# SheffieldML/GPy

Hardware: AMD Instinct MI355X
Metric: exact-GP log_lik+grad iters/sec (higher is better)
Workload: dtype f64; 1 GPU; BASELINE configs[2]: matern52 ARD exact GP, one GPRegression.parameters_changed, N=16384 D=32 Dy=1 per GPU; N=16384, D=32, kernel=matern52, ARD=True, parallelism=replicas x1

## Files before the change

### gpy_amd/_lib.py

```python
import ctypes
import os
import subprocess

import numpy as np
from numpy.ctypeslib import ndpointer

_HERE = os.path.dirname(os.path.abspath(__file__))
LIB_PATH = os.environ.get("MI355GP_LIB") or os.path.join(_HERE, "libmi355gp.so")
CSRC = os.path.join(_HERE, "csrc")

KIND_IDS = {"rbf": 0, "matern52": 1, "matern32": 2, "exponential": 3, "white": 4, "bias": 5, "ratquad": 6, "stdperiodic": 7,
            "coregionalize": 8, "linear": 9, "mlp": 10, "poly": 11, "cosine": 12, "sinc": 13, "expquadcosine": 14}


def ard_id(kind, ARD):
    if kind == "coregionalize":
        return int(ARD)
    return int(ARD) & 3 if kind == "stdperiodic" else int(bool(ARD))


class Part(ctypes.Structure):
    _fields_ = [("kind", ctypes.c_int), ("ard", ctypes.c_int), ("n_active", ctypes.c_int),
                ("active_dims", ctypes.POINTER(ctypes.c_int)), ("theta", ctypes.POINTER(ctypes.c_double)),
                ("term", ctypes.c_int)]
# ... 118 lines not shown
    "mi355gp_sparse_get_predict_ms": [_vp, _c_dp],
    "mi355gp_sparse_fetch_dLdKnm": [_vp, _i64, _i64, _dp],
    "mi355gp_sparse_attach_comm": [_vp, _ci, _ci, _str],
    "mi355gp_sparse_attach_loopback": [_vp, _ci, _ci, _ci],
    "mi355gp_sparse_fetch": [_vp, _ci, _dp],
    "mi355gp_sparse_get_profile": [_vp, _dp],
    "mi355gp_svgp_forward": [_vp, _ci, _parts, _dp, _i64, _dp, _dp, _ci, _cd, _dp, _dp, _dp, _c_dp],
    "mi355gp_svgp_backward": [_vp, _dp, _dp] + [_c_dp] * 5,
    "mi355gp_svgp_predict": [_vp, _ci, _parts, _c_dp, _i64, _ci] + [_c_dp] * 4,
    "mi355gp_pep_inference": [_vp, _ci, _parts, _dp, _i64, _cd, _cd, _cd, _dp] + [_c_dp] * 5,
    "mi355gp_pep_check_sigma": [_dp, _i64, _i64, _cd, _cd],
    "mi355gp_rbf_psi": [_ci, _cd, _dp, _ci, _dp, _i64, _dp, _dp, _i64, _ci] + [_c_dp] * 3,
    "mi355gp_rbf_psi_grad": [_ci, _cd, _dp, _ci, _dp, _i64, _dp, _dp, _i64, _ci] + [_c_dp] * 4 + [_dp] * 5,
    "mi355gp_bench_factor": [_ci, _i64, _ci, _c_dp, _c_dp, _c_dp],
    "mi355gp_dbg_ipc_selftest": [_str, _ci, _ci, _ci, _ci, _i64, _dp],
    "mi355gp_dbg_comm_selftest": [_ci, _str, _ci, _ci, _ci, _ci, _i64, _ci, _dp],
    "mi355gp_dbg_grid_multi": [_ci, _ci, _ci, _ci, _dp],
    "mi355gp_dbg_update_nt": [_ci, _ci, _ip, _ci, _ci, _dp],
    "mi355gp_dbg_update_rect": [_ci, _ci, _ci, _ip, _ci, _ci, _dp],
    "mi355gp_dbg_mfma": [_ci, _dp, _dp, _dp],
    "mi355gp_dbg_gemm": [_ci, _ci, _ci, _i64, _i64, _i64, _dp, _dp, _dp, _cd, _cd, _ci, _c_dp],
    "mi355gp_dbg_peaks": [_ci, _dp],
    "mi355gp_dbg_gemm_clock": [_c_dp, _c_dp],
    "mi355gp_dbg_cu_map": [_ci, _ci, _ci, ctypes.POINTER(ctypes.c_uint)],
    "mi355gp_dbg_pipe_share": [_ci, _dp],
    "mi355gp_dbg_graph_factor": [_ci, _i64, _ci, _dp],
    "mi355gp_dbg_persist": [_ci, _i64, _ci, _ci, _dp],
    "mi355gp_dbg_lauum_plan": [_ci, _ip, _ci, _ip],
    "mi355gp_dbg_persist_owners": [_ci, _ci, _ci, _ip, _ip],
    "mi355gp_dbg_mask_probe": [_ci, _ci, _ci, _dp],
}
EXPORTED = tuple(ABI)


def _opt(a):
    return None if a is None else a.ctypes.data_as(_c_dp)


def lib():
    global _lib
    if _lib is None:
        if not os.path.exists(LIB_PATH):
            build()
        L = ctypes.CDLL(LIB_PATH)
        for name, argtypes in ABI.items():
            getattr(L, name).argtypes = argtypes
        L.mi355gp_last_error.restype = L.mi355gp_version.restype = _str
        _lib = L
    return _lib


OPTIONS = {"profile": 0, "lookahead": 1, "tri_overlap": 2, "tri_min_nt": 3, "tri_h": 4, "tri_wgs": 5, "tri_half": 6,
           "part1_on_panel": 7, "nbo": 8, "solve_overlap": 9, "diag_excl_first": 10, "graph": 11, "persist": 12, "agg2": 13,
           "persist_test": 14, "persist_aborts": 15, "persist_skip": 16, "persist_sched": 17}


def last_error():
    return lib().mi355gp_last_error().decode()


def check(rc, what):
    if rc < 0:
        raise MI355GPError("%s failed (rc=%d): %s" % (what, rc, last_error()))
    return rc


def device_count():
    n = ctypes.c_int(0)
    lib().mi355gp_device_count(ctypes.byref(n))
    return n.value


def device_synchronize(device=0):
    require_device(device)
    check(lib().mi355gp_device_synchronize(int(device)), "mi355gp_device_synchronize")


def require_device(device=0):
    n = device_count()
    if device >= n:
        raise MI355GPError("no MI355X visible to HIP (device %d requested, %d present): the gpy_amd backend has "
                           "no CPU fallback" % (device, n))


def f64(a):
    return np.ascontiguousarray(a, dtype=np.float64)


def theta_vec(variance, lengthscale, ARD, D):
    ls = np.atleast_1d(np.asarray(lengthscale, dtype=np.float64)).ravel()
    if ARD:
        if ls.size == 1:
            ls = np.full(D, ls[0])
        assert ls.size == D, "ARD kernel needs one lengthscale per input dimension"
    else:
        assert ls.size == 1, "isotropic kernel has a single lengthscale"
    return np.concatenate([[float(np.asarray(variance).ravel()[0])], ls])


def _exact_result(out, ms, **arrays):
    res = dict(lml=out[OUT_LML], logdet=out[OUT_LOGDET], datafit=out[OUT_DATAFIT], dnoise=out[OUT_DNOISE],
               trKinv=out[OUT_TRKINV], **arrays)
    if ms is not None:
        res["stage_ms"] = dict(zip(STAGE_NAMES, ms[:len(STAGE_NAMES)]))
    return res


# ... 604 lines not shown
```

### gpy_amd/csrc/api.hip

```cpp
#include <cstdarg>
#include <cstdio>
#include <climits>
#include <string>
#include <vector>

#include "ctx.h"

static thread_local std::string g_err;

void mi355gp_set_error(const char* fmt, ...) {
    char buf[1024];
    va_list ap;
    va_start(ap, fmt);
    vsnprintf(buf, sizeof(buf), fmt, ap);
    va_end(ap);
    g_err = buf;
}

void apply_options(mi355gp_ctx* c) {
    FactorWs& w = c->ws;
    auto set = [&](int o, int* field) { if (c->opt[o] != INT_MIN) *field = c->opt[o]; };
    set(MI355GP_OPT_LOOKAHEAD, &w.lookahead);
    set(MI355GP_OPT_TRI_OVERLAP, &w.tri_overlap);
    set(MI355GP_OPT_TRI_MIN_NT, &w.tri_min_nt);
    set(MI355GP_OPT_TRI_H, &w.tri_h_override);
    set(MI355GP_OPT_TRI_WGS, &w.tri_wgs);
    set(MI355GP_OPT_TRI_HALF, &w.tri_half_ok);
    set(MI355GP_OPT_PART1_ON_PANEL, &w.part1_on_panel);
    set(MI355GP_OPT_NBO, &w.nbo_override);
    set(MI355GP_OPT_SOLVE_OVERLAP, &w.solve_overlap);
    set(MI355GP_OPT_DIAG_EXCL_FIRST, &w.diag_excl_first);
    set(MI355GP_OPT_PERSIST, &w.persist);
    set(MI355GP_OPT_AGG2, &w.agg2);
    if (c->opt[MI355GP_OPT_GRAPH] != INT_MIN) c->graph_enabled = c->opt[MI355GP_OPT_GRAPH] ? 1 : 0;
}

void drop_graph(mi355gp_ctx* c) {
    if (c->fgraph) (void)hipGraphExecDestroy(c->fgraph);
    c->fgraph = nullptr;
    c->fgraph_calls = 0;
}

void free_data(mi355gp_ctx* c) {
    drop_graph(c);
    c->parts.clear();
    double** ptrs[] = {&c->dX, &c->dR, &c->dNoise, &c->A, &c->B, &c->C, &c->Mbuf,
                       &c->dTmp, &c->dTrmvPart, &c->dGradPart, &c->dGradOut, &c->dPack, &c->dCoregPart};
    for (auto p : ptrs) {
        if (*p) (void)hipFree(*p);
        *p = nullptr;
    }
    if (c->hPack) (void)hipHostFree(c->hPack);
    c->hPack = nullptr;
    c->dAlpha = c->dScal = c->dDiag = c->dGradOutAll = nullptr;
    c->hIdx.clear();
    c->hIdxCol = -1;
    laplace_session_free(c->lap);
    c->lap = nullptr;
    c->lap_stage = 0;
    factor_ws_free(&c->ws);
    c->have_factor = c->have_kernel = false;
}

int ctx_prepare_parts(mi355gp_ctx* c, int nparts, const mi355gp_part* parts) {
    ARG_CHECK(nparts >= 1 && nparts <= 16 && parts, "between 1 and 16 kernel parts");
    if ((int)c->parts.size() != nparts) {
        c->parts.clear();
        c->parts.resize((size_t)nparts);
        for (auto& p : c->parts) HIP_CHECK(p.dXt.alloc((size_t)c->D * c->npad));
    }
    for (int i = 0; i < nparts; ++i) {
        mi355gp_ctx::Part& p = c->parts[(size_t)i];
        if (int rc = parse_part(parts[i], c->D, KS_STATIONARY | KS_STATIC | KS_EXT | KS_COREG | KS_LINEAR | KS_DOT | KS_OSC, "exact-GP path", &p)) return rc;
        if (p.coreg()) {
            const int col = p.kp.col;
            if (c->hIdxCol != col) {
                c->hIdx.resize((size_t)c->n);
                HIP_CHECK(hipMemcpy2D(c->hIdx.data(), sizeof(double), c->dX + col, sizeof(double) * c->D, sizeof(double), c->n,
                                      hipMemcpyDeviceToHost));
                c->hIdxCol = col;
            }
            if (int rc = coreg_check_index(c->hIdx.data(), c->n, 1, p.kp.ard, "training")) return rc;
            if (!c->dCoregPart) HIP_CHECK(hipMalloc(&c->dCoregPart, sizeof(double) * grad_num_blocks(c->n) * COREG_REC));
        }
        if (int rc = p.upload(c->st)) return rc;
    }
// ... 200 lines not shown
    }
    HIP_CHECK(hipMemcpyAsync(out, tmp, sizeof(double) * n * n, hipMemcpyDeviceToHost, st));
    HIP_CHECK(hipStreamSynchronize(st));
    return 0;
}

int mi355gp_set_option(mi355gp_ctx* c, int option, int value) {
    ARG_CHECK(c != nullptr, "mi355gp_set_option: NULL context");
    if (option == MI355GP_OPT_PROFILE) {
        c->ws.prof.on = (value != 0);
        c->ws.prof.mask = (value == 1) ? 0xffu : (unsigned)value >> 1;
        return 0;
    }
    if (option == MI355GP_OPT_PERSIST_TEST) {
#ifndef MI355GP_DIAG
        if (value != 0) {
            mi355gp_set_error("mi355gp_set_option: MI355GP_OPT_PERSIST_TEST is a test hook of the diagnostics build (libmi355gp_diag.so)");
            return -1;
        }
#endif
        c->ws.persist_test = value;
        if (value) c->ws.persist_skip = 0;
        drop_graph(c);
        return 0;
    }
    if (option < 0 || option >= MI355GP_OPT_NUM || option == MI355GP_OPT_PERSIST_ABORTS || option == MI355GP_OPT_PERSIST_SKIP ||
        option == MI355GP_OPT_PERSIST_SCHED) {
        mi355gp_set_error("mi355gp_set_option: unknown or read-only option %d", option);
        return -1;
    }
    if (option == MI355GP_OPT_LOOKAHEAD) value = (value == 0) ? 0 : 1;
    if (option == MI355GP_OPT_NBO && value > 0 && value % NB != 0) {
        mi355gp_set_error("mi355gp_set_option: NBO must be a multiple of %d", NB);
        return -1;
    }
    c->opt[option] = (value < 0) ? INT_MIN : value;
    if (value < 0) {
        FactorWs d;
#define env(name, dflt) diag_env_int(DIAG_ENV(name), dflt)
#define penv(name, dflt) diag_env_int(PRODUCT_ENV(name), dflt)
        switch (option) {
            case MI355GP_OPT_LOOKAHEAD: c->ws.lookahead = d.lookahead; break;
            case MI355GP_OPT_TRI_OVERLAP: c->ws.tri_overlap = penv("TRI_OVERLAP", d.tri_overlap) ? 1 : 0; break;
            case MI355GP_OPT_TRI_MIN_NT: c->ws.tri_min_nt = env("TRI_MIN_NT", d.tri_min_nt); break;
            case MI355GP_OPT_TRI_H: c->ws.tri_h_override = env("TRI_H", d.tri_h_override); break;
            case MI355GP_OPT_TRI_WGS: c->ws.tri_wgs = env("TRI_WGS", d.tri_wgs); break;
            case MI355GP_OPT_TRI_HALF: c->ws.tri_half_ok = env("TRI_HALF", d.tri_half_ok) ? 1 : 0; break;
            case MI355GP_OPT_PART1_ON_PANEL: c->ws.part1_on_panel = env("PART1_ON_PANEL", d.part1_on_panel) ? 1 : 0; break;
            case MI355GP_OPT_NBO: c->ws.nbo_override = env("NBO", d.nbo_override); break;
            case MI355GP_OPT_SOLVE_OVERLAP: c->ws.solve_overlap = env("SOLVE_OVERLAP", d.solve_overlap) ? 1 : 0; break;
            case MI355GP_OPT_DIAG_EXCL_FIRST: c->ws.diag_excl_first = env("DIAG_EXCL_FIRST", d.diag_excl_first) ? 1 : 0; break;
            case MI355GP_OPT_PERSIST: c->ws.persist = penv("PERSIST", d.persist); break;
            case MI355GP_OPT_AGG2: c->ws.agg2 = env("AGG2", d.agg2) ? 1 : 0; break;
            case MI355GP_OPT_GRAPH: c->graph_enabled = penv("GRAPH", 1) ? 1 : 0; break;
            default: break;
        }
#undef env
#undef penv
    }
    if (option == MI355GP_OPT_PERSIST) {
        c->ws.persist_auto_off = 0;
        c->ws.sched_force_steps = 0;
        c->ws.sched_np = c->ws.sched_ns = 0;
        c->ws.sched_state = (value < 0) ? 0 : 2;
    }
    apply_options(c);
    drop_graph(c);
    return 0;
}

int mi355gp_get_option(mi355gp_ctx* c, int option, int* value) {
    ARG_CHECK(c && value && option > MI355GP_OPT_PROFILE && option < MI355GP_OPT_NUM, "mi355gp_get_option: bad arguments");
    const FactorWs& w = c->ws;
    const int v[MI355GP_OPT_NUM] = {0, w.lookahead, w.tri_overlap, w.tri_min_nt, w.tri_h_override, w.tri_wgs, w.tri_half_ok,
                                    w.part1_on_panel, w.nbo_override, w.solve_overlap, w.diag_excl_first, c->graph_enabled,
                                    w.persist, w.agg2, w.persist_test, w.persist_aborts, w.persist_skip,
                                    w.sched_state == 2 ? ((w.persist_auto_off || !w.persist) ? 2 : 1) : 0};
    *value = v[option];
    return 0;
}

int mi355gp_get_profile(mi355gp_ctx* c, double* ms, double* flops, int* launches) {
    ARG_CHECK(c && ms && flops && launches, "mi355gp_get_profile: NULL argument");
    HIP_CHECK(hipSetDevice(c->device));
    HIP_CHECK(hipStreamSynchronize(c->st));
    if (c->ws.st_panel) HIP_CHECK(hipStreamSynchronize(c->ws.st_panel));
    if (c->ws.prof.collect(ms, flops, launches) != 0) {
        mi355gp_set_error("mi355gp_get_profile: event timing failed");
        return -5;
    }
    return 0;
}

}
```

### gpy_amd/csrc/factor.hip

```cpp
#include <cstdlib>
#include <mutex>
#include <vector>

#include "internal.h"

void KernelProf::begin(hipStream_t st, int fam, double flops) {
    open = on && ((mask >> fam) & 1u);
    if (!open) return;
    const size_t e0 = 2 * recs.size();
    while (pool.size() < e0 + 2) {
        hipEvent_t e;
        (void)hipEventCreate(&e);
        pool.push_back(e);
    }
    recs.push_back(Rec{fam, flops, e0});
    (void)hipEventRecord(pool[e0], st);
}

void KernelProf::end(hipStream_t st) {
    if (!open) return;
    open = false;
    (void)hipEventRecord(pool[recs.back().e0 + 1], st);
}

// ... 71 lines not shown
            void* touch = nullptr;
            if (hipMalloc(&touch, 256) == hipSuccess) {
                hipStream_t order[4] = {e.main, e.panel, e.tri, e.tri_half};
                for (hipStream_t s : order)
                    if (s) {
                        (void)hipMemsetAsync(touch, 0, 256, s);
                        (void)hipStreamSynchronize(s);
                    }
                (void)hipFree(touch);
            }
        }
        e.ready = true;
    }
    if (main) *main = e.main;
    if (panel) *panel = e.panel;
    if (tri) *tri = e.tri;
    if (tri_half) *tri_half = e.tri_half;
    return 0;
}

static bool lauum_plan_wanted(const FactorWs* ws, int nt);
static bool lauum_plan_build(FactorWs* ws, int nt);
int factor_ws_alloc(FactorWs* ws, long npad) {
    ws->nblk = npad / NB;
    HIP_CHECK(hipMalloc(&ws->dinv, sizeof(double) * ws->nblk * 8 * 256));
    HIP_CHECK(hipMalloc(&ws->logsum, sizeof(double) * ws->nblk));
    HIP_CHECK(hipMalloc(&ws->info, sizeof(int) * 4));
    int least = 0, greatest = 0;
    HIP_CHECK(hipDeviceGetStreamPriorityRange(&least, &greatest));
    int dev = 0;
    HIP_CHECK(hipGetDevice(&dev));
    if (factor_engine(dev, nullptr, &ws->st_panel, &ws->st_tri, &ws->st_tri_half) != 0) return -1;
    {
        const char* envo = PRODUCT_ENV("TRI_OVERLAP");
        if (envo && *envo) ws->tri_overlap = atoi(envo) ? 1 : 0;
        const char* envn2 = DIAG_ENV("TRI_MIN_NT");
        if (envn2 && *envn2) ws->tri_min_nt = atoi(envn2);
        const char* envw2 = DIAG_ENV("TRI_WGS");
        if (envw2 && *envw2) ws->tri_wgs = atoi(envw2);
        ws->tri_cu_pct = g_engine[dev].tri_pct > 0 && g_engine[dev].tri_pct <= 100 ? g_engine[dev].tri_pct : 75;
        HIP_CHECK(hipEventCreateWithFlags(&ws->ev_tri, hipEventDisableTiming));
        HIP_CHECK(hipEventCreateWithFlags(&ws->ev_tri_lead, hipEventDisableTiming));
        HIP_CHECK(hipMalloc(&ws->tri_counter, sizeof(int) * 4));
        const char* envh = DIAG_ENV("TRI_H");
        if (envh && *envh) ws->tri_h_override = atoi(envh);
    }
    const char* envp1 = DIAG_ENV("PART1_ON_PANEL");
    if (envp1 && *envp1) ws->part1_on_panel = atoi(envp1) ? 1 : 0;
    ws->sched_state = ws->sched_force_steps = ws->persist_auto_off = 0;
    ws->sched_np = ws->sched_ns = 0;
    ws->evals_done = ws->early_pending = 0;
    const char* envpa = PRODUCT_ENV("PERSIST_AUTO");
    if (envpa && *envpa) ws->persist_auto = atoi(envpa) ? 1 : 0;
    const char* envls = DIAG_ENV("LAUUM_SPLIT");
    if (envls && *envls) ws->lauum_split = atoi(envls) > 0 ? atoi(envls) : 0;
    const char* envptri = DIAG_ENV("PERSIST_TRI");
    if (envptri && *envptri) ws->persist_tri = atoi(envptri) ? 1 : 0;
    const char* envptn = DIAG_ENV("PERSIST_TRI_MIN_NT");
    if (envptn && *envptn) ws->persist_tri_min_nt = atoi(envptn);
#ifdef MI355GP_DIAG
    const char* envuq = DIAG_ENV("DBG_UPD_QUEUE");
    if (envuq && *envuq && atoi(envuq)) {
        ws->upd_queue_probe = 1;
        HIP_CHECK(hipMalloc(&ws->upd_tasks, sizeof(UpdTask) * 64 + 64));
    }
#endif
    const char* envag = DIAG_ENV("AGG2");
    if (envag && *envag) ws->agg2 = atoi(envag) ? 1 : 0;
    const char* envnbo = DIAG_ENV("NBO");
    if (envnbo && *envnbo) ws->nbo_override = atoi(envnbo);
    const char* envso = DIAG_ENV("SOLVE_OVERLAP");
    if (envso && *envso) ws->solve_overlap = atoi(envso) ? 1 : 0;
    const char* envth = DIAG_ENV("TRI_HALF");
    if (envth && *envth) ws->tri_half_ok = atoi(envth) ? 1 : 0;
    const char* envps = PRODUCT_ENV("PERSIST");
    if (envps && *envps) ws->persist = atoi(envps);
    const char* envpm = DIAG_ENV("PERSIST_MAX_NT");
    if (envpm && *envpm) ws->persist_max_nt = atoi(envpm);
    const char* envpt = DIAG_ENV("PERSIST_TUNE");
    if (envpt && *envpt) ws->persist_tune = atoi(envpt);
    const char* envpk = DIAG_ENV("PERSIST_KCAP");
    if (envpk && *envpk) ws->persist_kcap = atoi(envpk) > 0 ? atoi(envpk) : 1;
    {
        hipDeviceProp_t prop;
        HIP_CHECK(hipGetDeviceProperties(&prop, dev));
        ws->persist_cus = prop.multiProcessorCount;
        const char* envpc = DIAG_ENV("PERSIST_WGS");
        if (envpc && *envpc && atoi(envpc) >= 2 && atoi(envpc) <= ws->persist_cus) ws->persist_cus = atoi(envpc);
        HIP_CHECK(hipMalloc(&ws->persist_sync, sizeof(int) * potrf_persist_sync_ints()));
        HIP_CHECK(hipMalloc(&ws->persist_hs, sizeof(double) * (size_t)(ws->nblk < 64 ? ws->nblk : 64) * NB * NB));
    }
    const char* envx = DIAG_ENV("DIAG_EXCL_FIRST");
    if (envx && *envx) ws->diag_excl_first = atoi(envx) ? 1 : 0;
    HIP_CHECK(hipEventCreateWithFlags(&ws->ev_fork, hipEventDisableTiming));
    HIP_CHECK(hipEventCreateWithFlags(&ws->ev_early_pre, hipEventDisableTiming));
    if (lauum_plan_wanted(ws, (int)ws->nblk)) (void)lauum_plan_build(ws, (int)ws->nblk);
    const size_t nouter = (size_t)(npad + NB - 1) / NB + 2;
    ws->ev_panel.resize(nouter);
    ws->ev_cols.resize(nouter);
    for (size_t i = 0; i < nouter; ++i) {
        HIP_CHECK(hipEventCreateWithFlags(&ws->ev_panel[i], hipEventDisableTiming));
        HIP_CHECK(hipEventCreateWithFlags(&ws->ev_cols[i], hipEventDisableTiming));
    }
    return 0;
}

// ... 4 lines not shown
    ws->dinv = ws->logsum = nullptr;
    ws->info = nullptr;
    for (hipEvent_t e : ws->ev_panel) (void)hipEventDestroy(e);
    for (hipEvent_t e : ws->ev_cols) (void)hipEventDestroy(e);
    ws->ev_panel.clear();
    ws->ev_cols.clear();
    if (ws->ev_fork) (void)hipEventDestroy(ws->ev_fork);
    ws->ev_fork = nullptr;
    if (ws->ev_early_pre) (void)hipEventDestroy(ws->ev_early_pre);
    ws->ev_early_pre = nullptr;
    ws->st_panel = nullptr;
    ws->st_tri = nullptr;
    ws->st_tri_half = ws->st_tri_cur = nullptr;
    if (ws->ev_tri) (void)hipEventDestroy(ws->ev_tri);
    ws->ev_tri = nullptr;
    if (ws->ev_tri_lead) (void)hipEventDestroy(ws->ev_tri_lead);
    ws->ev_tri_lead = nullptr;
    if (ws->tri_counter) (void)hipFree(ws->tri_counter);
    ws->tri_counter = nullptr;
    if (ws->upd_tasks) (void)hipFree(ws->upd_tasks);
    ws->upd_tasks = nullptr;
    if (ws->lauum_plan_dev) (void)hipFree(ws->lauum_plan_dev);
    ws->lauum_plan_dev = nullptr;
    if (ws->lauum_part) (void)hipFree(ws->lauum_part);
    ws->lauum_part = nullptr;
    ws->lauum_plan_nt = 0;
    if (ws->persist_sync) (void)hipFree(ws->persist_sync);
    ws->persist_sync = nullptr;
    if (ws->persist_hs) (void)hipFree(ws->persist_hs);
    ws->persist_hs = nullptr;
    ws->prof.destroy();
}

static double syrk_flops(double n, double K) { return K * n * (n + 1.0); }
static double gemm_flops(double m, double n, double K) { return 2.0 * m * n * K; }

static void factor_panel(hipStream_t s, double* A, long npad, long K0, long W, FactorWs* ws) {
    const long ld = npad;
    for (long j = 0; j < W; j += NB) {
        const long c = K0 + j, blk = c / NB;
        double* dv = ws->dinv + blk * 8 * 256;
        ws->prof.begin(s, PF_DIAG, (double)NB * NB * NB / 3.0);
        launch_diag128(s, A, ld, c, dv, ws->logsum + blk, ws->info,
                       ws->diag_excl_first && c == K0 && ws->lookahead == 1 && ws->excl_first_ok);
        ws->prof.end(s);
        const long below = npad - (c + NB);
        if (below <= 0) continue;
        ws->prof.begin(s, PF_TRSM, (double)below * NB * NB);
        launch_trsm128(s, A, ld, c, c + NB, below, dv);
        ws->prof.end(s);
        const long cd = c + NB, ncols = K0 + W - cd;
        if (ncols <= 0) continue;
        const double* P = A + cd * ld + c;
        ws->prof.begin(s, update_nt_uses_64((int)(below / NB), (int)(ncols / NB), (int)(cd / NB), (int)(cd / NB)) ? PF_UPDATE64 : PF_UPDATE,
                       syrk_flops((double)ncols, (double)NB) + gemm_flops((double)(below - ncols), (double)ncols, (double)NB));
        launch_update_nt(s, A + cd * ld + cd, ld, P, ld, P, ld, NB, (int)(below / NB), (int)(ncols / NB), (int)(cd / NB), (int)(cd / NB));
        ws->prof.end(s);
    }
}

static void update_cols(hipStream_t s, double* A, long npad, long K0, long W, long c0, long c1, FactorWs* ws) {
    if (c1 <= c0) return;
    const long ld = npad, rows = npad - c0, cols = c1 - c0;
    const double* P = A + c0 * ld + K0;
    ws->prof.begin(s, update_nt_uses_64((int)(rows / NB), (int)(cols / NB), (int)(c0 / NB), (int)(c0 / NB)) ? PF_UPDATE64 : PF_UPDATE,
                   syrk_flops((double)cols, (double)W) + gemm_flops((double)(rows - cols), (double)cols, (double)W));
    launch_update_nt(s, A + c0 * ld + c0, ld, P, ld, P, ld, (int)W, (int)(rows / NB), (int)(cols / NB), (int)(c0 / NB),
                     (int)(c0 / NB));
    ws->prof.end(s);
}

static void potrf_serial(hipStream_t st, double* A, long npad, FactorWs* ws) {
    (void)hipMemsetAsync(ws->info, 0, sizeof(int) * 4, st);
    const long nbo = ws->nbo_for(npad);
    const long P = (npad + nbo - 1) / nbo;
    auto pcol = [&](long p) { return (p * nbo < npad) ? p * nbo : npad; };
    for (long p = 0; p < P; ++p) {
        factor_panel(st, A, npad, pcol(p), pcol(p + 1) - pcol(p), ws);
        update_cols(st, A, npad, pcol(p), pcol(p + 1) - pcol(p), pcol(p + 1), npad, ws);
    }
}

static void early_inverse(hipStream_t sq, double* A, long npad, int h, FactorWs* ws, bool gated, int gate_gives_up = 0) {
    const int ntl = (int)(npad / NB);
    (void)hipMemsetAsync(ws->tri_counter, 0, sizeof(int) * 4, sq);
    if (gated) launch_wait_persist_rows(sq, ws, 0, h, 0, gate_gives_up);
    ws->prof.begin(sq, PF_TRTRI_EARLY, 0.0);
    launch_inv128(sq, A, ws->scratchX, npad, h, ws->dinv);
    int level = 0;
    for (; (1 << level) < h; ++level) launch_trtri_level(sq, A, ws->scratchX, ws->scratchT, npad, h, level);
    (void)hipEventRecord(ws->ev_tri_lead, sq);
    const int nt_pair = ntl < 2 * h ? ntl : 2 * h;
    if (gated) launch_wait_persist_rows(sq, ws, h, nt_pair, h);
    launch_trtri_stage1_steal(sq, A, ws->scratchX, ws->scratchT, npad, nt_pair, level, ws->tri_counter,
                              ws->tri_wgs > 0 ? ws->tri_wgs : 512 * ws->tri_cur_pct / 100);
    ws->prof.end(sq);
    (void)hipEventRecord(ws->ev_tri, sq);
    ws->early_pending = 1;
}

int persist_early_h(long npad, const FactorWs* ws) {
    const int ntl = (int)(npad / NB);
    if (!potrf_persist_eligible(npad, ws) || !ws->tri_overlap || !ws->persist_tri || !ws->st_tri || !ws->scratchX || !ws->scratchT ||
        ntl < ws->persist_tri_min_nt || ws->evals_done < 1)
        return 0;
    int h = 1;
    static const int two_thirds = diag_env_int(DIAG_ENV("PERSIST_TRI_H23"), 1);
    if (two_thirds) while (6 * h <= 2 * ntl) h *= 2;
    else while (4 * h <= ntl) h *= 2;
    return h;
}

void calibrate_schedule(FactorWs& w, float ms, int nt) {
    if (w.sched_state == 0 && w.persist_used && w.evals_done >= 3) {
        w.sched_ms_persist = (w.sched_np == 0 || ms < w.sched_ms_persist) ? ms : w.sched_ms_persist;
        if (++w.sched_np >= 2) {
            w.sched_state = 1;
            w.sched_force_steps = 3;
            w.sched_ns = 0;
        }
    } else if (w.sched_state == 1 && !w.persist_used) {
// ... 221 lines not shown
```

### gpy_amd/csrc/gemm.hip

```cpp
#include "gemm_tile.h"
#include "internal.h"

#define LDS_OPT_IN(kernel)                                                                              \
    do {                                                                                                \
        static bool done = false;                                                                       \
        if (!done) {                                                                                    \
            (void)hipFuncSetAttribute(reinterpret_cast<const void*>(kernel),                            \
                                      hipFuncAttributeMaxDynamicSharedMemorySize, GT_LDS_BYTES);        \
            done = true;                                                                                \
        }                                                                                               \
    } while (0)

#include <algorithm>
#include <cstdlib>
#include <vector>
#define env_int(name, dflt) diag_env_int(DIAG_ENV(name), dflt)
#define LB(NW) __launch_bounds__((NW) * 64, (NW) / 2)

template <int NW, bool PRE>
__global__ LB(NW) void k_update_nt(double* __restrict__ C, long ldc,
                                                      const double* __restrict__ A, long lda,
                                                      const double* __restrict__ B, long ldb, int K, int ntc,
                                                      int row0t, int col0t, int tri, long ntiles) {
    extern __shared__ __attribute__((aligned(16))) double smem[];
    for (long bid = blockIdx.x; bid < ntiles; bid += gridDim.x) {
        int ti, tj;
        if (tri) {
            ti = (int)((sqrtf(8.0f * (float)bid + 1.0f) - 1.0f) * 0.5f);
            while ((long)ti * (ti + 1) / 2 > bid) --ti;
            while ((long)(ti + 1) * (ti + 2) / 2 <= bid) ++ti;
            tj = (int)(bid - (long)ti * (ti + 1) / 2);
        } else {
            ti = (int)(bid / ntc);
            tj = (int)(bid - (long)ti * ntc);
            if (col0t + tj > row0t + ti) continue;
        }
        d4 acc[4][GTCfg<NW>::NI];
        double* Ct = C + (long)ti * NB * ldc + (long)tj * NB;
        if (PRE) {
            gt_load_buf<NW>(Ct, ldc, acc);
            gemm_tile_128<true, true, NW, true>(A + (long)ti * NB * lda, lda, B + (long)tj * NB * ldb, ldb, K, acc, smem);
            gt_store<0, NW>(Ct, ldc, acc);
        } else {
            gt_zero<NW>(acc);
            gemm_tile_128<true, true, NW>(A + (long)ti * NB * lda, lda, B + (long)tj * NB * ldb, ldb, K, acc, smem);
            gt_store<2, NW>(Ct, ldc, acc);
        }
    }
}

__global__ __launch_bounds__(256) void k_update_nt64(double* __restrict__ C, long ldc, const double* __restrict__ A, long lda,
                                                     const double* __restrict__ B, long ldb, int K, int ntc, int row0t,
                                                     int col0t, int tri) {
    extern __shared__ __attribute__((aligned(16))) double smem[];
    const long bid = blockIdx.x >> 2;
    const int qi = (blockIdx.x >> 1) & 1, qj = blockIdx.x & 1;
    int ti, tj;
    if (tri) {
        ti = (int)((sqrtf(8.0f * (float)bid + 1.0f) - 1.0f) * 0.5f);
        while ((long)ti * (ti + 1) / 2 > bid) --ti;
        while ((long)(ti + 1) * (ti + 2) / 2 <= bid) ++ti;
        tj = (int)(bid - (long)ti * (ti + 1) / 2);
    } else {
        ti = (int)(bid / ntc);
        tj = (int)(bid - (long)ti * ntc);
        if (col0t + tj > row0t + ti) return;
    }
    d4 acc[2][2];
    double* Ct = C + ((long)ti * NB + qi * 64) * ldc + (long)tj * NB + qj * 64;
    gt64_load(Ct, ldc, acc);
    gemm_tile_64_v3<true, true, true>(A + ((long)ti * NB + qi * 64) * lda, lda, B + ((long)tj * NB + qj * 64) * ldb, ldb, K,
                                      acc, smem);
    gt64_store<0>(Ct, ldc, acc);
}

bool update_nt_uses_64(int ntr, int ntc, int row0t, int col0t) {
    static const int upd64_max = env_int("UPD64_MAX", GEMM_DEFAULT_UPD64_MAX);
    const int tri = (row0t == col0t && ntr == ntc) ? 1 : 0;
    const long nblocks = tri ? (long)ntr * (ntr + 1) / 2 : (long)ntr * ntc;
    return nblocks <= upd64_max;
}

void launch_update_nt(hipStream_t st, double* C, long ldc, const double* A, long lda, const double* B, long ldb,
                      int K, int ntr, int ntc, int row0t, int col0t) {
    if (ntr <= 0 || ntc <= 0) return;
    const int tri = (row0t == col0t && ntr == ntc) ? 1 : 0;
    const long nblocks = tri ? (long)ntr * (ntr + 1) / 2 : (long)ntr * ntc;
    if (update_nt_uses_64(ntr, ntc, row0t, col0t)) {
        hipLaunchKernelGGL(k_update_nt64, dim3((unsigned)(4 * nblocks)), dim3(256), GT64_LDS_BYTES, st, C, ldc, A, lda, B, ldb,
                           K, ntc, row0t, col0t, tri);
        return;
    }
    LDS_OPT_IN((k_update_nt<4, true>));
    hipLaunchKernelGGL((k_update_nt<4, true>), dim3((unsigned)nblocks), dim3(256), GT_LDS_BYTES, st, C, ldc, A, lda, B, ldb, K,
                       ntc, row0t, col0t, tri, nblocks);
}

#ifdef MI355GP_DIAG
__global__ LB(4) void k_update_nt_queue(double* __restrict__ A, long ld, const UpdTask* __restrict__ tasks, int ntasks,
                                        int* __restrict__ counter) {
    extern __shared__ __attribute__((aligned(16))) double smem[];
    __shared__ long s_tile;
    for (;;) {
        __syncthreads();
        if (threadIdx.x == 0) s_tile = (long)atomicAdd(counter, 1);
        __syncthreads();
        long bid = s_tile;
        int q = 0;
        while (q < ntasks && bid >= tasks[q].ntiles) bid -= tasks[q++].ntiles;
        if (q >= ntasks) return;
        const UpdTask tk = tasks[q];
        int ti = (int)((sqrtf(8.0f * (float)bid + 1.0f) - 1.0f) * 0.5f);
        while ((long)ti * (ti + 1) / 2 > bid) --ti;
        while ((long)(ti + 1) * (ti + 2) / 2 <= bid) ++ti;
        const int tj = (int)(bid - (long)ti * (ti + 1) / 2);
        d4 acc[4][GTCfg<4>::NI];
        double* Ct = A + tk.c_off + (long)ti * NB * ld + (long)tj * NB;
        const double* P = A + tk.p_off;
        gt_load_buf<4>(Ct, ld, acc);
        gemm_tile_128<true, true, 4, true>(P + (long)ti * NB * ld, ld, P + (long)tj * NB * ld, ld, tk.K, acc, smem);
        gt_store<0, 4>(Ct, ld, acc);
    }
}

void launch_update_nt_queue(hipStream_t st, double* A, long ld, const UpdTask* tasks_dev, int ntasks, int* counter, int wgs) {
    LDS_OPT_IN(k_update_nt_queue);
    hipLaunchKernelGGL(k_update_nt_queue, dim3((unsigned)wgs), dim3(256), GT_LDS_BYTES, st, A, ld, tasks_dev, ntasks, counter);
}
#endif

__host__ __device__ __forceinline__ int trtri_rows_last(int nt, int nbt) {
    const int pairs = (nt + 2 * nbt - 1) / (2 * nbt), right0 = (2 * (pairs - 1) + 1) * nbt;
    const int rows = nt - right0;
    return rows < 0 ? 0 : (rows > nbt ? nbt : rows);
}
__host__ __device__ __forceinline__ long trtri_level_tiles(int nt, int nbt) {
    const int pairs = (nt + 2 * nbt - 1) / (2 * nbt);
    return (long)(pairs - 1) * nbt * nbt + (long)nbt * trtri_rows_last(nt, nbt);
}
template <int STAGE>
__device__ __forceinline__ void trtri_map(int bid, int nt, int nbt, int& p, int& ri, int& cj) {
    const int per = nbt * nbt, pairs = (nt + 2 * nbt - 1) / (2 * nbt), full = (pairs - 1) * per;
    if (bid < full) {
// ... 493 lines not shown
```

### gpy_amd/csrc/internal.h

```cpp
#pragma once
#include <shared_mutex>
#include <vector>

#include "common.h"

bool update_nt_uses_64(int ntr, int ntc, int row0t, int col0t);
struct UpdTask { long c_off, p_off, ntiles; int K, ntr; };
#ifdef MI355GP_DIAG
void launch_update_nt_queue(hipStream_t st, double* A, long ld, const UpdTask* tasks_dev, int ntasks, int* counter, int wgs);
#endif
void launch_update_nt(hipStream_t st, double* C, long ldc, const double* A, long lda, const double* B, long ldb,
                      int K, int ntr, int ntc, int row0t, int col0t);
void launch_trtri_level(hipStream_t st, const double* L, double* X, double* T, long ld, int nt, int level,
                        int stages = 3);
void launch_lauum(hipStream_t st, const double* X, double* W, long ld, int nt);
struct LauumItem { int ti, tj, q, k0, klen, part; };
struct LauumSum { int ti, tj, q, first, n; };
void lauum_split_plan(int nt, std::vector<LauumItem>& items, std::vector<LauumSum>& sums, int* nparts);
int lauum_split_tile(int nt);
void launch_lauum_split(hipStream_t st, const double* X, double* W, long ld, int nt, const LauumItem* items_dev, int nitems,
                        const LauumSum* sums_dev, int nsums, double* part);
bool lauum_uses_64(int nt);
void launch_trmm_lower(hipStream_t st, const double* X, long ldx, const double* B, long ldb, double* Out, long ldo,
                       int ntr, int ntc);
void launch_trmm_lower_T(hipStream_t st, const double* X, long ldx, const double* B, long ldb, double* Out, long ldo,
                         int ntr, int ntc);
void launch_trmm64(hipStream_t st, int mode, const double* X, long ldx, const double* B, long ldb, double* Out, long ldo, int nt,
                   int ntother, double alpha);
void launch_gemm_tn_sq(hipStream_t st, const double* A, long lda, long K, double* C, long ldc, int nt, double alpha,
                       double beta);
void launch_dbg_gemm(hipStream_t st, int a_mcontig, int b_ncontig, long M, long N, long K, const double* A,
                     const double* B, double* C, double alpha, double beta);

void launch_diag128(hipStream_t st, double* A, long ld, long c0, double* dinv, double* logsum, int* info,
                    int exclusive = 0);
void launch_trsm128(hipStream_t st, double* A, long ld, long c0, long r0, long mrows, const double* dinv);
void launch_trtri_stage1_steal(hipStream_t st, const double* L, double* X, double* T, long ld, int nt, int level,
                               int* counter, int grid);
void launch_inv128(hipStream_t st, const double* L, double* X, long ld, int nblk, const double* dinv_all);
void launch_dbg_mfma(hipStream_t st, const double* a, const double* b, double* d);

enum { PF_UPDATE = 0, PF_TRTRI = 1, PF_LAUUM = 2, PF_DIAG = 3, PF_TRSM = 4, PF_UPDATE64 = 5, PF_PERSIST = 6, PF_TRTRI_EARLY = 7, PF_NUM = 8 };
struct KernelProf {
    unsigned mask = 0;
    bool on = false;
    std::vector<hipEvent_t> pool;
    struct Rec { int fam; double flops; size_t e0; };
    std::vector<Rec> recs;
    bool open = false;
    void begin(hipStream_t st, int fam, double flops);
    void end(hipStream_t st);
    void reset() { recs.clear(); }
    int collect(double* ms, double* flops, int* launches);
    void destroy();
};

struct FactorWs {
    double* dinv = nullptr;
    double* logsum = nullptr;
    int* info = nullptr;
    long nblk = 0;
    hipStream_t st_panel = nullptr;
    std::vector<hipEvent_t> ev_panel;
    std::vector<hipEvent_t> ev_cols;
    hipEvent_t ev_fork = nullptr;
    hipEvent_t ev_early_pre = nullptr;
    int agg2 = 0;
    int persist_auto = 1, sched_state = 0, sched_force_steps = 0, persist_auto_off = 0;
    int sched_np = 0, sched_ns = 0;
    int can_calibrate = 0;
    float sched_ms_persist = 0.f, sched_ms_steps = 0.f;
    int evals_done = 0;
    int early_pending = 0;
    int lauum_split = 1, lauum_plan_nt = 0, lauum_nitems = 0, lauum_nsums = 0;
    void* lauum_plan_dev = nullptr;
    double* lauum_part = nullptr;
    int persist_tri = 1;
    int persist_tri_min_nt = 16;
    int upd_queue_probe = 0;
    UpdTask* upd_tasks = nullptr;
    int part1_on_panel = 1;
    int lookahead = 1;
    int nbo_override = 0;
    long nbo_for(long npad) const {
        long w = nbo_override > 0 ? nbo_override : (npad <= FACTOR_NBO_SMALL_N ? FACTOR_NBO_SMALL : NBO);
        w = (w / NB) * NB;
        return w < NB ? NB : w;
    }
    double* scratchX = nullptr;
    double* scratchT = nullptr;
    int tri_overlap = FACTOR_DEFAULT_TRI_OVERLAP, tri_cu_pct = 75, tri_min_nt = 48, tri_wgs = 0, ovl_h = 0;
    hipStream_t st_tri = nullptr, st_tri_half = nullptr, st_tri_cur = nullptr;
    int tri_half_ok = 1, tri_cur_pct = 75;
    hipEvent_t ev_tri = nullptr, ev_tri_lead = nullptr;
    int* tri_counter = nullptr;
    int tri_h_override = 0;
    int diag_excl_first = FACTOR_DEFAULT_DIAG_EXCL_FIRST, excl_first_ok = 0;
    int solve_overlap = 1;
    int persist = FACTOR_DEFAULT_PERSIST, persist_max_nt = FACTOR_PERSIST_MAX_NT, persist_kcap = 2, persist_cus = 0;
    int persist_skip = 0, persist_aborts = 0, persist_used = 0;
    hipEvent_t ev_persist_pre = nullptr;
    int persist_grid_last = 0;
    int persist_tune = 0;
    int persist_test = 0;
    int* persist_sync = nullptr;
    double* persist_hs = nullptr;
    KernelProf prof;
};
std::shared_mutex& engine_gate(int device);
struct EngineShared {
    std::shared_mutex* m;
    bool shared = true;
    explicit EngineShared(int device) : m(&engine_gate(device)) { m->lock_shared(); }
    EngineShared(const EngineShared&) = delete;
    EngineShared& operator=(const EngineShared&) = delete;
    ~EngineShared() {
        if (shared) m->unlock_shared();
        else m->unlock();
    }
    bool try_exclusive() {
        m->unlock_shared();
        if (m->try_lock()) {
            shared = false;
            return true;
        }
        m->lock_shared();
        return false;
    }
    void share() {
        m->unlock();
        m->lock_shared();
        shared = true;
    }
// ... 129 lines not shown
```

### include/mi355gp.h

```cpp
#ifndef MI355GP_H
#define MI355GP_H

#include <stdint.h>

#ifdef __cplusplus
extern "C" {
#endif

typedef struct mi355gp_ctx mi355gp_ctx;

enum { MI355GP_RBF = 0, MI355GP_MATERN52 = 1, MI355GP_MATERN32 = 2, MI355GP_EXPONENTIAL = 3,
       MI355GP_WHITE = 4, MI355GP_BIAS = 5 ,
       MI355GP_RATQUAD = 6, MI355GP_STDPERIODIC = 7, MI355GP_COREGIONALIZE = 8, MI355GP_LINEAR = 9,
       MI355GP_MLP = 10, MI355GP_POLY = 11, MI355GP_COSINE = 12, MI355GP_SINC = 13, MI355GP_EXPQUADCOSINE = 14 };






typedef struct {
    int kind;
    int ard;
    int n_active;
// ... 50 lines not shown
                            double* diag_dLdK_out, double* stage_ms);

int mi355gp_exact_inference_sum(mi355gp_ctx* ctx, int nparts, const mi355gp_part* parts, const double* noise,
                                int64_t noise_len, double jitter, double extra_jitter, double* out_scalars,
                                double* alpha_out, double* dtheta_out, double* diag_dLdK_out, double* stage_ms);

int mi355gp_exact_studentt_sum(mi355gp_ctx* ctx, int nparts, const mi355gp_part* parts, double nu, double jitter,
                               double extra_jitter, double* out_scalars, double* alpha_out, double* dtheta_out,
                               double* stage_ms);

int mi355gp_inference_given_K(mi355gp_ctx* ctx, const double* K_host, const double* noise, int64_t noise_len,
                              double jitter, double extra_jitter, double* out_scalars, double* alpha_out,
                              double* diag_dLdK_out, double* stage_ms);

int mi355gp_fetch(mi355gp_ctx* ctx, int which, double* out, int fortran_order);

int mi355gp_predict(mi355gp_ctx* ctx, int kind, int ard, const double* theta, const double* Xnew, int64_t M,
                    double* mu_out, double* var_out, int full_cov);

int mi355gp_predict_sum(mi355gp_ctx* ctx, int nparts, const mi355gp_part* parts, const double* Xnew, int64_t M,
                        double* mu_out, double* var_out, int full_cov);

int mi355gp_predictive_gradients_sum(mi355gp_ctx* ctx, int nparts, const mi355gp_part* parts, const double* Xnew, int64_t M,
                                     double* dmu_out, double* dvar_out);

int mi355gp_laplace_begin(mi355gp_ctx* ctx, int nparts, const mi355gp_part* parts);
int mi355gp_laplace_newton(mi355gp_ctx* ctx, const double* W, const double* b, double extra_jitter, double* a_out,
                           double* Ka_out, double* logdet_out);
int mi355gp_laplace_finish(mi355gp_ctx* ctx, const double* W, double extra_jitter, double* diagKiWi_out, double* logdet_out);
int mi355gp_laplace_gradients(mi355gp_ctx* ctx, const double* Ki_f, const double* dL_dfhat, double* dtheta_out);
int mi355gp_laplace_implicit(mi355gp_ctx* ctx, const double* dL_dfhat, double* s_out);
int mi355gp_laplace_predict(mi355gp_ctx* ctx, int nparts, const mi355gp_part* parts, const double* Xnew, int64_t M,
                            const double* wv, double* mu_out, double* var_out, int full_cov);

enum { MI355GP_EP_BERNOULLI_PROBIT = 0 };
int mi355gp_ep_recompute(mi355gp_ctx* ctx, const double* tau, const double* v, double extra_jitter, double add_diag,
                         int want_sigma, double* mu_out, double* sigdiag_out, double* logdet_out, double* ms_out);
int mi355gp_ep_sweep(mi355gp_ctx* ctx, int lik, const int64_t* order, const double* ysign, double eta, double delta, double* tau,
                     double* v, double* cav_tau_out, double* cav_v_out, double* logZhat_out, double* mu_out, double* sigdiag_out,
                     double* ms_out);

int mi355gp_covariance_between_points(mi355gp_ctx* ctx, int nparts, const mi355gp_part* parts, const double* X1,
                                      int64_t M1, const double* X2, int64_t M2, double* out);

int mi355gp_potrf(int device, double* A, int64_t N, double* ms);
int mi355gp_pdinv(int device, const double* A, int64_t N, double* Ainv, double* L_out, double* logdet, double* ms);
int mi355gp_pdinv_full(int device, const double* A, int64_t N, double* Ainv, double* L_out, double* Li_out, double* logdet,
                       double* ms);

enum { MI355GP_OPT_PROFILE = 0, MI355GP_OPT_LOOKAHEAD = 1, MI355GP_OPT_TRI_OVERLAP = 2, MI355GP_OPT_TRI_MIN_NT = 3,
       MI355GP_OPT_TRI_H = 4, MI355GP_OPT_TRI_WGS = 5, MI355GP_OPT_TRI_HALF = 6, MI355GP_OPT_PART1_ON_PANEL = 7,
       MI355GP_OPT_NBO = 8, MI355GP_OPT_SOLVE_OVERLAP = 9, MI355GP_OPT_DIAG_EXCL_FIRST = 10, MI355GP_OPT_GRAPH = 11,
       MI355GP_OPT_PERSIST = 12, MI355GP_OPT_AGG2 = 13, MI355GP_OPT_PERSIST_TEST = 14, MI355GP_OPT_PERSIST_ABORTS = 15,
       MI355GP_OPT_PERSIST_SKIP = 16, MI355GP_OPT_PERSIST_SCHED = 17, MI355GP_OPT_NUM = 18 };
int mi355gp_set_option(mi355gp_ctx* ctx, int option, int value);
int mi355gp_get_option(mi355gp_ctx* ctx, int option, int* value);
enum { MI355GP_PF_UPDATE = 0 , MI355GP_PF_TRTRI = 1, MI355GP_PF_LAUUM = 2,
       MI355GP_PF_DIAG = 3 , MI355GP_PF_TRSM = 4 ,
       MI355GP_PF_UPDATE64 = 5 ,
       MI355GP_PF_PERSIST = 6 ,
       MI355GP_PF_TRTRI_EARLY = 7 ,
       MI355GP_PF_NUM = 8 };
int mi355gp_get_profile(mi355gp_ctx* ctx, double* ms, double* flops, int* launches);

typedef struct mi355gp_grid mi355gp_grid;
int mi355gp_grid_unique_id(void* id128);
int mi355gp_grid_create(int device, int rank, int world, int Pr, int Pc, int nb, const void* id128, mi355gp_grid** out);
int mi355gp_grid_destroy(mi355gp_grid* g);
int mi355gp_grid_set_data(mi355gp_grid* g, const double* X, int64_t N, int D, const double* R, int Dy);
int mi355gp_grid_exact_inference(mi355gp_grid* g, int kind, int ard, const double* theta, const double* noise,
                                 int64_t noise_len, double jitter, double extra_jitter, double* out_scalars,
                                 double* alpha_out, double* dtheta_out, double* diag_dLdK_out, double* stage_ms);
#define MI355GP_FETCH_LINV 100
int mi355gp_grid_fetch(mi355gp_grid* g, int which, double* out);
enum { MI355GP_GRID_OPT_LOOKAHEAD = 0, MI355GP_GRID_OPT_G = 1, MI355GP_GRID_OPT_GW = 2, MI355GP_GRID_OPT_CHECK_SEQ = 3,
       MI355GP_GRID_OPT_NUM = 4 };
int mi355gp_grid_set_option(mi355gp_grid* g, int option, int value);
int mi355gp_grid_get_option(mi355gp_grid* g, int option, int* value);
int mi355gp_grid_coll_log(mi355gp_grid* g, int rank, double* out9);
typedef struct mi355gp_sparse mi355gp_sparse;
int mi355gp_sparse_create(int device, mi355gp_sparse** out);
int mi355gp_sparse_destroy(mi355gp_sparse* s);
int mi355gp_sparse_set_data(mi355gp_sparse* s, const double* X, int64_t N, int D, const double* Y, int Dy);
int mi355gp_vardtc_inference(mi355gp_sparse* s, int kind, int ard, const double* theta, const double* Z, int64_t M,
                             double noise_var, double extra_jitter, double* out_scalars, double* dtheta_out,
                             double* dZ_out, double* wv_out, double* stage_ms);
int mi355gp_vardtc_inference_sum(mi355gp_sparse* s, int nparts, const mi355gp_part* parts, const double* Z, int64_t M,
                                 const double* noise, int64_t noise_len, double extra_jitter, double* out_scalars,
                                 double* dtheta_out, double* dZ_out, double* wv_out, double* dnoise_rows_out,
                                 double* dLdm_out, double* stage_ms);
int mi355gp_sparse_set_input_variance(mi355gp_sparse* s, const double* S, int64_t N, int D);
int mi355gp_sparse_set_inputs(mi355gp_sparse* s, const double* X, const double* S, int64_t N, int D);
int mi355gp_vardtc_inference_uncertain(mi355gp_sparse* s, int nparts, const mi355gp_part* parts, const double* Z, int64_t M,
                                       const double* noise, int64_t noise_len, double extra_jitter, double* out_scalars,
                                       double* dtheta_out, double* dZ_out, double* wv_out, double* dmu_out, double* dS_out,
                                       double* stage_ms);
int mi355gp_sparse_predict(mi355gp_sparse* s, int nparts, const mi355gp_part* parts, const double* Xnew, int64_t Mn,
                           double* mu_out, double* var_out, int full_cov);
int mi355gp_sparse_predict_uncertain(mi355gp_sparse* s, int nparts, const mi355gp_part* parts, const double* mu_new,
                                     const double* S_new, int64_t Mn, double* mean_out, double* var_out);
int mi355gp_sparse_get_predict_ms(mi355gp_sparse* s, double* ms_out);
int mi355gp_sparse_fetch_dLdKnm(mi355gp_sparse* s, int64_t row0, int64_t nrows, double* out);
int mi355gp_sparse_attach_comm(mi355gp_sparse* s, int rank, int world, const void* id128);
int mi355gp_sparse_attach_loopback(mi355gp_sparse* s, int rank, int world, int group_key);
int mi355gp_sparse_fetch(mi355gp_sparse* s, int which, double* out);
int mi355gp_sparse_get_profile(mi355gp_sparse* s, double* out6);

// ... 26 lines not shown
```

Measured before the change: 14.01 iters/s.

## Split tail of Cholesky trailing update into quarter tiles to balance last wave

Adds a mixed-granularity trailing-update kernel in which the last nquad 128x128 tiles are each split into four 64x64 sub-tiles. A small cost model picks nquad from the tile count, K and the number of CU slots so the final partial wave is filled more evenly. The goal is to cut the idle time on compute units during the tail of each blocked Cholesky update. In exchange it adds per-shape planning (memoised), a second code path inside one kernel, and hard-coded timing constants in the model that may not fit every shape.

Result: no change. 13.98 iters/s (-0.2%).

```diff
diff --git a/gpy_amd/_lib.py b/gpy_amd/_lib.py
--- a/gpy_amd/_lib.py
+++ b/gpy_amd/_lib.py
@@ -194,7 +194,7 @@
 
 OPTIONS = {"profile": 0, "lookahead": 1, "tri_overlap": 2, "tri_min_nt": 3, "tri_h": 4, "tri_wgs": 5, "tri_half": 6,
            "part1_on_panel": 7, "nbo": 8, "solve_overlap": 9, "diag_excl_first": 10, "graph": 11, "persist": 12, "agg2": 13,
-           "persist_test": 14, "persist_aborts": 15, "persist_skip": 16, "persist_sched": 17}
+           "persist_test": 14, "persist_aborts": 15, "persist_skip": 16, "persist_sched": 17, "upd_mix": 18}
 
 
 def last_error():
diff --git a/gpy_amd/csrc/api.hip b/gpy_amd/csrc/api.hip
--- a/gpy_amd/csrc/api.hip
+++ b/gpy_amd/csrc/api.hip
@@ -32,6 +32,7 @@
     set(MI355GP_OPT_DIAG_EXCL_FIRST, &w.diag_excl_first);
     set(MI355GP_OPT_PERSIST, &w.persist);
     set(MI355GP_OPT_AGG2, &w.agg2);
+    set(MI355GP_OPT_UPD_MIX, &w.upd_mix);
     if (c->opt[MI355GP_OPT_GRAPH] != INT_MIN) c->graph_enabled = c->opt[MI355GP_OPT_GRAPH] ? 1 : 0;
 }
 
@@ -338,6 +339,7 @@
             case MI355GP_OPT_DIAG_EXCL_FIRST: c->ws.diag_excl_first = env("DIAG_EXCL_FIRST", d.diag_excl_first) ? 1 : 0; break;
             case MI355GP_OPT_PERSIST: c->ws.persist = penv("PERSIST", d.persist); break;
             case MI355GP_OPT_AGG2: c->ws.agg2 = env("AGG2", d.agg2) ? 1 : 0; break;
+            case MI355GP_OPT_UPD_MIX: c->ws.upd_mix = env("UPD_MIX", d.upd_mix) < 0 ? -1 : env("UPD_MIX", d.upd_mix); break;
             case MI355GP_OPT_GRAPH: c->graph_enabled = penv("GRAPH", 1) ? 1 : 0; break;
             default: break;
         }
@@ -361,7 +363,7 @@
     const int v[MI355GP_OPT_NUM] = {0, w.lookahead, w.tri_overlap, w.tri_min_nt, w.tri_h_override, w.tri_wgs, w.tri_half_ok,
                                     w.part1_on_panel, w.nbo_override, w.solve_overlap, w.diag_excl_first, c->graph_enabled,
                                     w.persist, w.agg2, w.persist_test, w.persist_aborts, w.persist_skip,
-                                    w.sched_state == 2 ? ((w.persist_auto_off || !w.persist) ? 2 : 1) : 0};
+                                    w.sched_state == 2 ? ((w.persist_auto_off || !w.persist) ? 2 : 1) : 0, w.upd_mix};
     *value = v[option];
     return 0;
 }
diff --git a/gpy_amd/csrc/factor.hip b/gpy_amd/csrc/factor.hip
--- a/gpy_amd/csrc/factor.hip
+++ b/gpy_amd/csrc/factor.hip
@@ -147,6 +147,10 @@
     ws->evals_done = ws->early_pending = 0;
     const char* envpa = PRODUCT_ENV("PERSIST_AUTO");
     if (envpa && *envpa) ws->persist_auto = atoi(envpa) ? 1 : 0;
+    const char* envum = DIAG_ENV("UPD_MIX");
+    if (envum && *envum) ws->upd_mix = atoi(envum) < 0 ? -1 : atoi(envum);
+    const char* envla = DIAG_ENV("LOOKAHEAD");
+    if (envla && *envla) ws->lookahead = atoi(envla) ? 1 : 0;
     const char* envls = DIAG_ENV("LAUUM_SPLIT");
     if (envls && *envls) ws->lauum_split = atoi(envls) > 0 ? atoi(envls) : 0;
     const char* envptri = DIAG_ENV("PERSIST_TRI");
@@ -257,9 +261,10 @@
         const long cd = c + NB, ncols = K0 + W - cd;
         if (ncols <= 0) continue;
         const double* P = A + cd * ld + c;
-        ws->prof.begin(s, update_nt_uses_64((int)(below / NB), (int)(ncols / NB), (int)(cd / NB), (int)(cd / NB)) ? PF_UPDATE64 : PF_UPDATE,
+        ws->prof.begin(s, update_nt_uses_64((int)(below / NB), (int)(ncols / NB), (int)(cd / NB), (int)(cd / NB), ws->upd_mix) ? PF_UPDATE64 : PF_UPDATE,
                        syrk_flops((double)ncols, (double)NB) + gemm_flops((double)(below - ncols), (double)ncols, (double)NB));
-        launch_update_nt(s, A + cd * ld + cd, ld, P, ld, P, ld, NB, (int)(below / NB), (int)(ncols / NB), (int)(cd / NB), (int)(cd / NB));
+        launch_update_nt(s, A + cd * ld + cd, ld, P, ld, P, ld, NB, (int)(below / NB), (int)(ncols / NB), (int)(cd / NB), (int)(cd / NB),
+                         ws->upd_mix);
         ws->prof.end(s);
     }
 }
@@ -268,10 +273,10 @@
     if (c1 <= c0) return;
     const long ld = npad, rows = npad - c0, cols = c1 - c0;
     const double* P = A + c0 * ld + K0;
-    ws->prof.begin(s, update_nt_uses_64((int)(rows / NB), (int)(cols / NB), (int)(c0 / NB), (int)(c0 / NB)) ? PF_UPDATE64 : PF_UPDATE,
+    ws->prof.begin(s, update_nt_uses_64((int)(rows / NB), (int)(cols / NB), (int)(c0 / NB), (int)(c0 / NB), ws->upd_mix) ? PF_UPDATE64 : PF_UPDATE,
                    syrk_flops((double)cols, (double)W) + gemm_flops((double)(rows - cols), (double)cols, (double)W));
     launch_update_nt(s, A + c0 * ld + c0, ld, P, ld, P, ld, (int)W, (int)(rows / NB), (int)(cols / NB), (int)(c0 / NB),
-                     (int)(c0 / NB));
+                     (int)(c0 / NB), ws->upd_mix);
     ws->prof.end(s);
 }
 
diff --git a/gpy_amd/csrc/gemm.hip b/gpy_amd/csrc/gemm.hip
--- a/gpy_amd/csrc/gemm.hip
+++ b/gpy_amd/csrc/gemm.hip
@@ -13,7 +13,10 @@
 
 #include <algorithm>
 #include <cstdlib>
+#include <mutex>
 #include <vector>
+
+#include "upd_mix_plan.h"
 #define env_int(name, dflt) diag_env_int(DIAG_ENV(name), dflt)
 #define LB(NW) __launch_bounds__((NW) * 64, (NW) / 2)
 
@@ -74,21 +77,87 @@
     gt64_store<0>(Ct, ldc, acc);
 }
 
-bool update_nt_uses_64(int ntr, int ntc, int row0t, int col0t) {
+__global__ LB(4) void k_update_nt_mix(double* __restrict__ C, long ldc, const double* __restrict__ A, long lda,
+                                      const double* __restrict__ B, long ldb, int K, int ntc, int row0t, int col0t, int tri,
+                                      long nfull) {
+    extern __shared__ __attribute__((aligned(16))) double smem[];
+    const bool quad = (long)blockIdx.x >= nfull;
+    const long q = quad ? (long)blockIdx.x - nfull : 0;
+    const long bid = quad ? nfull + (q >> 2) : (long)blockIdx.x;
+    int ti, tj;
+    if (tri) {
+        ti = (int)((sqrtf(8.0f * (float)bid + 1.0f) - 1.0f) * 0.5f);
+        while ((long)ti * (ti + 1) / 2 > bid) --ti;
+        while ((long)(ti + 1) * (ti + 2) / 2 <= bid) ++ti;
+        tj = (int)(bid - (long)ti * (ti + 1) / 2);
+    } else {
+        ti = (int)(bid / ntc);
+        tj = (int)(bid - (long)ti * ntc);
+        if (col0t + tj > row0t + ti) return;
+    }
+    if (!quad) {
+        d4 acc[4][GTCfg<4>::NI];
+        double* Ct = C + (long)ti * NB * ldc + (long)tj * NB;
+        gt_load_buf<4>(Ct, ldc, acc);
+        gemm_tile_128<true, true, 4, true>(A + (long)ti * NB * lda, lda, B + (long)tj * NB * ldb, ldb, K, acc, smem);
+        gt_store<0, 4>(Ct, ldc, acc);
+    } else {
+        const int qi = (int)(q >> 1) & 1, qj = (int)q & 1;
+        d4 acc[2][2];
+        double* Ct = C + ((long)ti * NB + qi * 64) * ldc + (long)tj * NB + qj * 64;
+        gt64_load(Ct, ldc, acc);
+        gemm_tile_64_v3<true, true, true>(A + ((long)ti * NB + qi * 64) * lda, lda, B + ((long)tj * NB + qj * 64) * ldb, ldb, K,
+                                          acc, smem);
+        gt64_store<0>(Ct, ldc, acc);
+    }
+}
+
+bool update_nt_uses_64(int ntr, int ntc, int row0t, int col0t, int mix) {
     static const int upd64_max = env_int("UPD64_MAX", GEMM_DEFAULT_UPD64_MAX);
     const int tri = (row0t == col0t && ntr == ntc) ? 1 : 0;
     const long nblocks = tri ? (long)ntr * (ntr + 1) / 2 : (long)ntr * ntc;
-    return nblocks <= upd64_max;
+    return mix <= 0 && nblocks <= upd64_max;
+}
+
+static int update_slots() {
+    static int slots[16] = {};
+    int dev = 0;
+    if (hipGetDevice(&dev) != hipSuccess || dev < 0 || dev >= 16) return 512;
+    if (!slots[dev]) {
+        int ncu = 0;
+        if (hipDeviceGetAttribute(&ncu, hipDeviceAttributeMultiprocessorCount, dev) != hipSuccess || ncu <= 0) ncu = 256;
+        slots[dev] = 2 * ncu;
+    }
+    return slots[dev];
+}
+
+static long update_mix_nquad(long T, int K, int slots) {
+    struct Key { long T; int K, slots; long nquad; };
+    static std::vector<Key> memo;
+    static std::mutex m;
+    std::lock_guard<std::mutex> lock(m);
+    for (const Key& k : memo)
+        if (k.T == T && k.K == K && k.slots == slots) return k.nquad;
+    const long nquad = upd_mix_plan(T, K, slots);
+    if (memo.size() < 4096) memo.push_back(Key{T, K, slots, nquad});
+    return nquad;
 }
 
 void launch_update_nt(hipStream_t st, double* C, long ldc, const double* A, long lda, const double* B, long ldb,
-                      int K, int ntr, int ntc, int row0t, int col0t) {
+                      int K, int ntr, int ntc, int row0t, int col0t, int mix) {
     if (ntr <= 0 || ntc <= 0) return;
     const int tri = (row0t == col0t && ntr == ntc) ? 1 : 0;
     const long nblocks = tri ? (long)ntr * (ntr + 1) / 2 : (long)ntr * ntc;
-    if (update_nt_uses_64(ntr, ntc, row0t, col0t)) {
+    if (update_nt_uses_64(ntr, ntc, row0t, col0t, mix)) {
         hipLaunchKernelGGL(k_update_nt64, dim3((unsigned)(4 * nblocks)), dim3(256), GT64_LDS_BYTES, st, C, ldc, A, lda, B, ldb,
                            K, ntc, row0t, col0t, tri);
+        return;
+    }
+    const long nquad = mix > 0 ? (mix < nblocks ? (long)mix : nblocks) : mix < 0 ? update_mix_nquad(nblocks, K, update_slots()) : 0;
+    if (nquad > 0) {
+        LDS_OPT_IN(k_update_nt_mix);
+        hipLaunchKernelGGL(k_update_nt_mix, dim3((unsigned)(nblocks + 3 * nquad)), dim3(256), GT_LDS_BYTES, st, C, ldc, A, lda, B,
+                           ldb, K, ntc, row0t, col0t, tri, nblocks - nquad);
         return;
     }
     LDS_OPT_IN((k_update_nt<4, true>));
diff --git a/gpy_amd/csrc/internal.h b/gpy_amd/csrc/internal.h
--- a/gpy_amd/csrc/internal.h
+++ b/gpy_amd/csrc/internal.h
@@ -4,13 +4,13 @@
 
 #include "common.h"
 
-bool update_nt_uses_64(int ntr, int ntc, int row0t, int col0t);
+bool update_nt_uses_64(int ntr, int ntc, int row0t, int col0t, int mix = -1);
 struct UpdTask { long c_off, p_off, ntiles; int K, ntr; };
 #ifdef MI355GP_DIAG
 void launch_update_nt_queue(hipStream_t st, double* A, long ld, const UpdTask* tasks_dev, int ntasks, int* counter, int wgs);
 #endif
 void launch_update_nt(hipStream_t st, double* C, long ldc, const double* A, long lda, const double* B, long ldb,
-                      int K, int ntr, int ntc, int row0t, int col0t);
+                      int K, int ntr, int ntc, int row0t, int col0t, int mix = -1);
 void launch_trtri_level(hipStream_t st, const double* L, double* X, double* T, long ld, int nt, int level,
                         int stages = 3);
 void launch_lauum(hipStream_t st, const double* X, double* W, long ld, int nt);
@@ -79,6 +79,7 @@
     int persist_tri_min_nt = 16;
     int upd_queue_probe = 0;
     UpdTask* upd_tasks = nullptr;
+    int upd_mix = -1;
     int part1_on_panel = 1;
     int lookahead = 1;
     int nbo_override = 0;
diff --git a/gpy_amd/csrc/upd_mix_plan.h b/gpy_amd/csrc/upd_mix_plan.h
--- /dev/null
+++ b/gpy_amd/csrc/upd_mix_plan.h
@@ -0,0 +1,47 @@
+#pragma once
+#include <algorithm>
+#include <functional>
+#include <queue>
+#include <vector>
+
+static inline double upd_mix_last_round_us(long n, int slots, double one, double two) {
+    return n <= 0 ? 0.0 : (2 * n <= slots ? one : two);
+}
+
+static inline double upd_mix_finish_us(long T, int K, int slots, long nquad) {
+    if (T <= 0 || slots <= 0) return 0.0;
+    nquad = std::min(std::max(nquad, 0L), T);
+    const double k = (double)K / 128.0;
+    const double tile2 = 27.4 * k + 8.0, tile1 = 13.7 * k + 8.0, quad2 = 27.4 * k / 4.0 + 8.0, quad1 = 13.7 * k / 4.0 + 8.0;
+    const long nfull = T - nquad, rounds = nfull / slots, rest = nfull % slots, nq = 4 * nquad;
+    if (nquad == 0) return (double)rounds * tile2 + upd_mix_last_round_us(rest, slots, tile1, tile2);
+    if (rest == 0) return (double)rounds * tile2 + (double)(nq / slots) * quad2 + upd_mix_last_round_us(nq % slots, slots, quad1, quad2);
+    std::priority_queue<double, std::vector<double>, std::greater<double>> slot;
+    for (long s = 0; s < slots; ++s) slot.push((double)(rounds + (s < rest ? 1 : 0)) * tile2);
+    double end = (double)(rounds + 1) * tile2;
+    for (long i = 0; i < nq; ++i) {
+        const double t = slot.top() + quad2;
+        slot.pop();
+        slot.push(t);
+        if (t > end) end = t;
+    }
+    return end;
+}
+
+static inline long upd_mix_plan(long T, int K, int slots, double* finish_us = nullptr) {
+    long best = 0;
+    double best_us = upd_mix_finish_us(T, K, slots, 0);
+    if (T > 0 && slots > 0 && T % slots != 0) {
+        const long r = T % slots;
+        for (int j = 0; j <= 8; ++j) {
+            const long n = std::min(r + (long)j * slots / 8, T);
+            const double us = upd_mix_finish_us(T, K, slots, n);
+            if (us < best_us - 0.5) {
+                best_us = us;
+                best = n;
+            }
+        }
+    }
+    if (finish_us) *finish_us = best_us;
+    return best;
+}
diff --git a/include/mi355gp.h b/include/mi355gp.h
--- a/include/mi355gp.h
+++ b/include/mi355gp.h
@@ -126,7 +126,7 @@
        MI355GP_OPT_TRI_H = 4, MI355GP_OPT_TRI_WGS = 5, MI355GP_OPT_TRI_HALF = 6, MI355GP_OPT_PART1_ON_PANEL = 7,
        MI355GP_OPT_NBO = 8, MI355GP_OPT_SOLVE_OVERLAP = 9, MI355GP_OPT_DIAG_EXCL_FIRST = 10, MI355GP_OPT_GRAPH = 11,
        MI355GP_OPT_PERSIST = 12, MI355GP_OPT_AGG2 = 13, MI355GP_OPT_PERSIST_TEST = 14, MI355GP_OPT_PERSIST_ABORTS = 15,
-       MI355GP_OPT_PERSIST_SKIP = 16, MI355GP_OPT_PERSIST_SCHED = 17, MI355GP_OPT_NUM = 18 };
+       MI355GP_OPT_PERSIST_SKIP = 16, MI355GP_OPT_PERSIST_SCHED = 17, MI355GP_OPT_UPD_MIX = 18, MI355GP_OPT_NUM = 19 };
 int mi355gp_set_option(mi355gp_ctx* ctx, int option, int value);
 int mi355gp_get_option(mi355gp_ctx* ctx, int option, int* value);
 enum { MI355GP_PF_UPDATE = 0 , MI355GP_PF_TRTRI = 1, MI355GP_PF_LAUUM = 2,
```
